# santi-pdp/segan_pytorch

Hardware: NVIDIA H100
Metric: 16384-sample windows/sec (G+D train step) (higher is better)
Workload: dtype f16 operands / f32 accumulate (f16 gradient tensors, loss scale 1024)

## Files before the change

include/segan_b200.h:

```cpp
#ifndef SEGAN_B200_H
#define SEGAN_B200_H

#include <stdint.h>

#ifdef __cplusplus
extern "C" {
#endif

#define SG_ABI_VERSION 3

#define SG_STAT_SLICES 8

#define SG_OK 0
#define SG_ERR_INVALID -1
#define SG_ERR_LAUNCH -2
#define SG_ERR_UNSUPPORTED -3

#define SG_F32 0
#define SG_F16 1
#define SG_BF16 2

#define SG_ACT_NONE 0
#define SG_ACT_PRELU 1
#define SG_ACT_TANH 2
// ... 33 lines not shown
  int32_t n_lo, n_hi;
  const float* bias;
  int32_t bias_mod;
  int32_t batch;
  int32_t ksplit;
  int32_t backend;
  int32_t tile_n;
  double* bn_stats;
  void* out2;
  int32_t out2_halo;
  const float* slope;
  int32_t slope_mod;
  void* sk_ws;
} sg_tapgemm_f;

int sg_tapgemm_f_run(const sg_tapgemm_f* p, void* stream);
int64_t sg_tapgemm_f_workspace_bytes(void);
int sg_debug_timeline(unsigned long long* host_out, int max_words);

typedef struct sg_tapgemm_w {
  const void* g;
  int32_t g_rows, g_dtype;
  const void* a0;
  const void* a1;
  int32_t a0_c, a1_c;
  int32_t a_rows, a_halo, a_dtype;
  int32_t kc, nc;
  int32_t d_lo, d_hi;
  int32_t tap_k_lo[9], tap_k_hi[9], tap_n_lo[9], tap_n_hi[9];
  float* dw;
// ... 134 lines not shown
```

segan_pytorch_b200/csrc/tapgemm_tc.cu:

```cuda
#include "common.cuh"
#include <cuda.h>
#include <stdlib.h>

namespace sg {

__device__ __forceinline__ uint32_t smem_u32(const void* p) {
  return static_cast<uint32_t>(__cvta_generic_to_shared(p));
}
__device__ __forceinline__ void mbar_init(uint64_t* bar, uint32_t count) {
  asm volatile("mbarrier.init.shared::cta.b64 [%0], %1;" ::"r"(smem_u32(bar)), "r"(count));
}
__device__ __forceinline__ void mbar_expect_tx(uint64_t* bar, uint32_t bytes) {
  asm volatile("mbarrier.arrive.expect_tx.shared::cta.b64 _, [%0], %1;" ::"r"(smem_u32(bar)), "r"(bytes)
               : "memory");
}
__device__ __forceinline__ void mbar_arrive(uint64_t* bar) {
  asm volatile("mbarrier.arrive.shared::cta.b64 _, [%0];" ::"r"(smem_u32(bar)) : "memory");
}
__device__ __forceinline__ uint32_t mbar_try(uint32_t addr, uint32_t parity) {
  uint32_t done;
  asm volatile(
      "{\n"
      ".reg .pred p;\n"
      "mbarrier.try_wait.parity.shared::cta.b64 p, [%1], %2;\n"
// ... 52 lines not shown
  asm volatile("ld.shared.v4.b32 {%0, %1, %2, %3}, [%4];" : "=r"(v.x), "=r"(v.y), "=r"(v.z), "=r"(v.w) : "r"(addr) : "memory");
  return v;
}
__device__ __forceinline__ void red_add_v2(float* addr, float a, float b) {
  asm volatile("red.global.add.v2.f32 [%0], {%1, %2};" ::"l"(addr), "f"(a), "f"(b) : "memory");
}
__device__ __forceinline__ void wgmma_fence() { asm volatile("wgmma.fence.sync.aligned;" ::: "memory"); }
__device__ __forceinline__ void wgmma_commit() { asm volatile("wgmma.commit_group.sync.aligned;" ::: "memory"); }
template <int N>
__device__ __forceinline__ void wgmma_wait() { asm volatile("wgmma.wait_group.sync.aligned %0;" ::"n"(N) : "memory"); }
template <int R>
__device__ __forceinline__ void setmaxnreg_inc() { asm volatile("setmaxnreg.inc.sync.aligned.u32 %0;" ::"n"(R)); }
template <int R>
__device__ __forceinline__ void setmaxnreg_dec() { asm volatile("setmaxnreg.dec.sync.aligned.u32 %0;" ::"n"(R)); }
__device__ __forceinline__ void consumer_bar_sync() { asm volatile("bar.sync 1, 256;" ::: "memory"); }

template <int TA, int TB>
__device__ __forceinline__ void wgmma_f16_n64(float (&d)[32], uint64_t da, uint64_t db, int scale_d) {
  asm volatile(
      "{\n.reg .pred p;\nsetp.ne.b32 p, %34, 0;\n"
      "wgmma.mma_async.sync.aligned.m64n64k16.f32.f16.f16 "
      "{%0, %1, %2, %3, %4, %5, %6, %7, %8, %9, %10, %11, %12, %13, %14, %15, %16, %17, %18, %19, %20, %21, %22, %23, %24, %25, %26, %27, %28, %29, %30, %31}, %32, %33, p, 1, 1, %35, %36;\n}\n"
      : "+f"(d[0]), "+f"(d[1]), "+f"(d[2]), "+f"(d[3]), "+f"(d[4]), "+f"(d[5]), "+f"(d[6]), "+f"(d[7]), "+f"(d[8]), "+f"(d[9]), "+f"(d[10]), "+f"(d[11]), "+f"(d[12]), "+f"(d[13]), "+f"(d[14]), "+f"(d[15]), "+f"(d[16]), "+f"(d[17]), "+f"(d[18]), "+f"(d[19]), "+f"(d[20]), "+f"(d[21]), "+f"(d[22]), "+f"(d[23]), "+f"(d[24]), "+f"(d[25]), "+f"(d[26]), "+f"(d[27]), "+f"(d[28]), "+f"(d[29]), "+f"(d[30]), "+f"(d[31])
      : "l"(da), "l"(db), "r"(scale_d), "n"(TA), "n"(TB));
}

template <int TA, int TB>
__device__ __forceinline__ void wgmma_bf16_n64(float (&d)[32], uint64_t da, uint64_t db, int scale_d) {
  asm volatile(
      "{\n.reg .pred p;\nsetp.ne.b32 p, %34, 0;\n"
// ... 65 lines not shown
  d |= (uint64_t)((sbo_bytes >> 4) & 0x3FFF) << 32;
  d |= (uint64_t)1 << 62;
  return d;
}

template <int N, int TA, int TB, bool BF16>
__device__ __forceinline__ void mma_k64(float (&acc)[N / 2], uint64_t da, uint64_t db, uint32_t a_step,
                                        uint32_t b_step, bool first) {
  wgmma_fence();
#pragma unroll
  for (int kk = 0; kk < 4; ++kk)
    wgmma_tile<N, TA, TB, BF16>(acc, da + kk * a_step, db + kk * b_step, (first && kk == 0) ? 0 : 1);
  wgmma_commit();
}

constexpr int STAGES = 4;
constexpr int A_STAGE_BYTES = 128 * 128;
constexpr int B_STAGE_BYTES = 256 * 128;
constexpr int STAGE_BYTES = A_STAGE_BYTES + B_STAGE_BYTES;
constexpr int SMEM_BYTES = STAGES * STAGE_BYTES + 1024  + 256  + 2048 ;
constexpr int OUT_CHUNK_BYTES = 128 * 128;
constexpr int OUT_STAGE_OFF = STAGES * STAGE_BYTES;
constexpr int F_CTL_OFF = OUT_STAGE_OFF + 2 * OUT_CHUNK_BYTES;
constexpr int F_SMEM_BYTES = F_CTL_OFF + 256  + 1024 ;
static_assert(F_SMEM_BYTES <= 232448, "form-F shared memory exceeds the sm_90 opt-in limit");
constexpr int NUM_THREADS = 384;
constexpr int PRODUCER_REGS = 40, CONSUMER_REGS = 232;

struct TapRangesTC {
  int k_lo[NTAP], k_hi[NTAP], n_lo[NTAP], n_hi[NTAP];
};

struct FTcParams {
  int a0_c, kc, nc, a_halo;
  int d_lo, d_hi;
  TapRangesTC tr;
  void* out; int out_dtype, out_rows, out_halo, out_ld, out_col0;
  int w_tap0;
  int m_lo, m_hi, n_lo;
  const float* bias; int bias_mod;
  int batch, ksplit;
  int TR, TB, TN;
  int m_tiles_per_b, b_tiles, n_tiles;
  int dbg;
  double* stats;
  int sk_dp_tiles;
  int sk_split;
  float* sk_ws;
  unsigned int* sk_cnt;
  void* out2;
  int out2_halo;
  const float* slope; int slope_mod;
  int bias_mask, slope_mask;
  int tma_out;
};

struct SharedCtl {
  uint64_t full[STAGES];
  uint64_t empty[STAGES];
};

__device__ __forceinline__ int f_num_steps(const FTcParams& p, int n0, int ks) {
  int total = 0;
  for (int d = p.d_lo; d <= p.d_hi; ++d) {
    const int ti = d + 4;
    if (n0 + p.TN <= p.tr.n_lo[ti] || n0 >= p.tr.n_hi[ti]) continue;
    total += (p.tr.k_hi[ti] - p.tr.k_lo[ti]) >> 6;
  }
  return p.ksplit == 1 ? total : (total - ks + p.ksplit - 1) / p.ksplit;
}

struct Piece {
  int tile;
  int mt, rest;
  int kb, ke;
  int total;
};

constexpr int TL_SLOTS = 32;
constexpr int TL_CTAS = 160;
__device__ unsigned long long g_tc_timeline[TL_CTAS * TL_SLOTS];
__device__ __forceinline__ unsigned long long gtime_ns() {
  unsigned long long t;
  asm volatile("mov.u64 %0, %globaltimer;" : "=l"(t));
  return t;
}

struct PieceIter {
  int m_tiles, nctas, dp_end, total_tiles, cta;
  int next_dp, cur_mt, cur_rest;
  int cache_rest, cache_steps;
  bool sk_done;

  __device__ __forceinline__ int steps_of_rest(const FTcParams& p, int rest) {
    if (rest != cache_rest) {
      cache_rest = rest;
// ... 132 lines not shown
        sx += __shfl_xor_sync(0xffffffffu, sx, o);
        sy += __shfl_xor_sync(0xffffffffu, sy, o);
        qx += __shfl_xor_sync(0xffffffffu, qx, o);
        qy += __shfl_xor_sync(0xffffffffu, qy, o);
      }
      if (lane < 4) {
        atomicAdd(colstat + c, sx);
        atomicAdd(colstat + c + 1, sy);
        atomicAdd(colstat + 256 + c, qx);
        atomicAdd(colstat + 256 + c + 1, qy);
      }
    }
  }
}

template <int TN>
__device__ __forceinline__ void f_epilogue_tma(const FTcParams& p, const float (&acc)[TN / 2], int mt, int n0,
                                               int ctid, uint32_t stg, const CUtensorMap* tmO,
                                               const CUtensorMap* tmO2) {
  const int lane = ctid & 31, cw = ctid >> 5;
  const int mtb = p.m_tiles_per_b == 1 ? mt : mt / p.m_tiles_per_b;
  const int b0 = mtb * p.TB;
  const int m0 = p.m_lo + (mt - mtb * p.m_tiles_per_b) * p.TR;
  const bool two = p.out2 != nullptr;
  const bool act_in_place = p.slope != nullptr && !two;
  const bool add_bias = p.bias != nullptr;
  const uint32_t row_off = (uint32_t)(cw * 16 + (lane >> 2)) * 128u + 4u * (lane & 3);
  const int sw = lane >> 2;
  const int halo2 = p.out2_halo;
  const bool mirror_tile = two && halo2 > 0 &&
                           ((m0 <= halo2 && m0 + p.TR > 1) || (m0 + p.TR > p.out_rows - 1 - halo2 && m0 <= p.out_rows - 2));
  constexpr int NQ = TN / 64;
#pragma unroll
  for (int q = 0; q < NQ; ++q) {
    const bool round_start = two || (q & 1) == 0;
    const bool round_end = two || (q & 1) == 1 || q == NQ - 1;
    const uint32_t slot = stg + (two ? 0u : (uint32_t)(q & 1) * OUT_CHUNK_BYTES);
    if (round_start) {
      if (ctid == 0) bulk_wait_read_all();
      consumer_bar_sync();
    }
#pragma unroll
    for (int jj = 0; jj < 8; ++jj) {
      const int j = 8 * q + jj;
      const int c = 8 * j + 2 * (lane & 3);
      float bx = 0.f, by = 0.f;
      if (add_bias) {
        const float* bp = p.bias + f_mod(n0 + c, p.bias_mod, p.bias_mask);
        bx = __ldg(bp); by = __ldg(bp + 1);
      }
      float s0 = 0.f, s1 = 0.f;
      if (p.slope != nullptr) {
        const float* sp = p.slope + f_mod(n0 + c, p.slope_mod, p.slope_mask);
        s0 = __ldg(sp); s1 = __ldg(sp + 1);
      }
      const uint32_t col_off = (uint32_t)((jj ^ sw) << 4);
#pragma unroll
      for (int h = 0; h < 2; ++h) {
        float x = acc[4 * j + 2 * h] + bx, y = acc[4 * j + 2 * h + 1] + by;
        if (act_in_place) {
          x = x > 0.f ? x : s0 * x;
          y = y > 0.f ? y : s1 * y;
        }
        const uint32_t off = row_off + (uint32_t)h * 1024u + col_off;
        st_shared_u32(slot + off, pack2(x, y, p.out_dtype));
        if (two) st_shared_u32(slot + OUT_CHUNK_BYTES + off, pack2(x > 0.f ? x : s0 * x, y > 0.f ? y : s1 * y, p.out_dtype));
      }
    }
    if (!round_end) continue;
    fence_proxy_async_smem();
    consumer_bar_sync();
    if (ctid == 0) {
      const int c_rel = n0 - p.n_lo + 64 * q, m_rel = m0 - p.m_lo;
      if (two) {
        tma_store_3d(tmO, slot, c_rel, m_rel, b0);
        tma_store_3d(tmO2, slot + OUT_CHUNK_BYTES, c_rel, m_rel, b0);
      } else if (q & 1) {
        tma_store_3d(tmO, stg, c_rel - 64, m_rel, b0);
        tma_store_3d(tmO, stg + OUT_CHUNK_BYTES, c_rel, m_rel, b0);
      } else {
        tma_store_3d(tmO, stg, c_rel, m_rel, b0);
      }
      bulk_commit();
    }
    if (mirror_tile) {
      const int rows = p.TR * p.TB;
      const int out2_buf_rows = p.out_rows + 2 * halo2;
      for (int idx = ctid; idx < rows * 8; idx += 256) {
        const int r = idx >> 3, k = idx & 7;
        const int tb = r / p.TR, tr = r - tb * p.TR;
        const int b = b0 + tb, m = m0 + tr;
        if (b >= p.batch || m >= p.m_hi) continue;
        int mm;
        if (m >= 1 && m <= halo2) mm = -m;
        else if (m >= p.out_rows - 1 - halo2 && m <= p.out_rows - 2) mm = 2 * (p.out_rows - 1) - m;
        else continue;
        const uint4 v = ld_shared_v4(slot + OUT_CHUNK_BYTES + (uint32_t)r * 128u + (uint32_t)((k ^ (r & 7)) << 4));
        const int64_t o = ((int64_t)b * out2_buf_rows + halo2 + mm) * p.out_ld + p.out_col0 + (n0 - p.n_lo) + 64 * q + 8 * k;
        *reinterpret_cast<uint4*>(reinterpret_cast<uint16_t*>(p.out2) + o) = v;
      }
    }
  }
}

template <int TN, bool BF16>
__global__ void __launch_bounds__(NUM_THREADS, 1)
tapgemm_f_tc(const __grid_constant__ CUtensorMap tmA0, const __grid_constant__ CUtensorMap tmA1,
             const __grid_constant__ CUtensorMap tmW, const __grid_constant__ CUtensorMap tmO,
             const __grid_constant__ CUtensorMap tmO2, const FTcParams p) {
  extern __shared__ uint8_t smem_raw[];
  uint8_t* smem = reinterpret_cast<uint8_t*>((reinterpret_cast<uintptr_t>(smem_raw) + 1023) & ~uintptr_t(1023));
  SharedCtl* ctl = reinterpret_cast<SharedCtl*>(smem + F_CTL_OFF);
  float* colstat = reinterpret_cast<float*>(smem + OUT_STAGE_OFF);
  const int wg = threadIdx.x >> 7;

  if (threadIdx.x == 0) {
    prefetch_tmap(&tmA0); prefetch_tmap(&tmA1); prefetch_tmap(&tmW);
    if (p.tma_out) {
      prefetch_tmap(&tmO);
      if (p.out2 != nullptr) prefetch_tmap(&tmO2);
    }
    for (int s = 0; s < STAGES; ++s) { mbar_init(&ctl->full[s], 1); mbar_init(&ctl->empty[s], 2); }
    fence_barrier_init();
  }
  if (p.stats != nullptr)
    for (int c = threadIdx.x; c < 512; c += NUM_THREADS) colstat[c] = 0.f;
  __syncthreads();

  const int m_tiles = p.m_tiles_per_b * p.b_tiles;
  const int total_tiles = m_tiles * p.n_tiles * p.ksplit;
  const uint32_t a_bytes = (uint32_t)p.TR * p.TB * 128u;
  const uint32_t b_bytes = (uint32_t)TN * 128u;
  PieceIter it;
  it.init(p, m_tiles, total_tiles, blockIdx.x, gridDim.x);
  Piece pc;

  if (wg == 0) {
// ... 2 lines not shown
      int stage = 0; uint32_t phase = 0;
      while (it.next(p, pc)) {
        const int ks = p.ksplit == 1 ? 0 : pc.rest % p.ksplit;
        const int nt = p.ksplit == 1 ? pc.rest : pc.rest / p.ksplit;
        const int mtb = p.m_tiles_per_b == 1 ? pc.mt : pc.mt / p.m_tiles_per_b;
        const int b0 = mtb * p.TB;
        const int m0 = p.m_lo + (pc.mt - mtb * p.m_tiles_per_b) * p.TR;
        const int n0 = p.n_lo + nt * p.TN;
        const bool interleaved = p.ksplit > 1;
        int step = 0, sel = 0;
        int skip = interleaved ? 0 : pc.kb;
        int next_sel = ks;
        const int kstride = interleaved ? 64 * p.ksplit : 64;
        for (int d = p.d_lo; d <= p.d_hi; ++d) {
          const int ti = d + 4;
          if (n0 + p.TN <= p.tr.n_lo[ti] || n0 >= p.tr.n_hi[ti]) continue;
          const int klo = p.tr.k_lo[ti], khi = p.tr.k_hi[ti];
          const int nk = (khi - klo) >> 6;
          int k0 = klo;
          if (!interleaved) {
            if (skip >= nk) { skip -= nk; sel += nk; continue; }
            k0 += skip << 6; sel += skip; skip = 0;
            if (sel >= pc.ke) break;
          } else {
            if (next_sel >= step + nk) { step += nk; continue; }
            k0 += (next_sel - step) << 6;
          }
          for (; k0 < khi; k0 += kstride) {
            if (!interleaved) {
              if (sel++ >= pc.ke) break;
            } else {
              next_sel += p.ksplit;
            }
            mbar_wait(&ctl->empty[stage], phase ^ 1);
            uint8_t* sa = smem + stage * STAGE_BYTES;
            mbar_expect_tx(&ctl->full[stage], a_bytes + b_bytes);
            if (k0 < p.a0_c) tma_load_3d(sa, &tmA0, &ctl->full[stage], k0, m0 + d + p.a_halo, b0);
            else tma_load_3d(sa, &tmA1, &ctl->full[stage], k0 - p.a0_c, m0 + d + p.a_halo, b0);
            tma_load_2d(sa + A_STAGE_BYTES, &tmW, &ctl->full[stage], k0, (ti - p.w_tap0) * p.nc + n0);
            if (++stage == STAGES) { stage = 0; phase ^= 1; }
          }
          step += nk;
        }
      }
    }
    return;
  }

  setmaxnreg_inc<CONSUMER_REGS>();
  const int ctid = threadIdx.x - 128;
  const int cwg = wg - 1;
  const bool wg_leader = (threadIdx.x & 127) == 0;
  const uint32_t smem0 = smem_u32(smem);
  int stage = 0; uint32_t phase = 0;
  int stat_nt = -1;
  auto flush_stats = [&](int nt_done) {
    consumer_bar_sync();
    const int n0s = p.n_lo + nt_done * p.TN;
    double* o = p.stats + (int64_t)(blockIdx.x % SG_STAT_SLICES) * 2 * p.nc;
    for (int c = ctid; c < p.TN; c += 256) {
      atomicAdd(o + n0s + c, (double)colstat[c]);
      atomicAdd(o + p.nc + n0s + c, (double)colstat[256 + c]);
      colstat[c] = 0.f;
      colstat[256 + c] = 0.f;
    }
    consumer_bar_sync();
  };
  const bool tl_on = (p.dbg & (1 << 20)) && ctid == 0 && blockIdx.x < TL_CTAS;
  int tl_i = 0;
  unsigned long long* tl = g_tc_timeline + (blockIdx.x < TL_CTAS ? blockIdx.x : 0) * TL_SLOTS;
  if (tl_on) { for (int i = 0; i < TL_SLOTS; ++i) tl[i] = 0; tl[tl_i++] = gtime_ns(); }

  float acc[TN / 2];
  while (it.next(p, pc)) {
    const int ks = p.ksplit == 1 ? 0 : pc.rest % p.ksplit;
    const int nt = p.ksplit == 1 ? pc.rest : pc.rest / p.ksplit;
    const int n0 = p.n_lo + nt * p.TN;
    const bool partial = pc.tile >= it.dp_end;
    if (p.stats != nullptr && nt != stat_nt) {
      if (stat_nt >= 0) flush_stats(stat_nt);
      stat_nt = nt;
    }
    const int nsteps = pc.ke - pc.kb;
    if (nsteps == 0) {
#pragma unroll
      for (int j = 0; j < TN / 2; ++j) acc[j] = 0.f;
    }
    int prev = 0;
    for (int i = 0; i < nsteps; ++i) {
      mbar_wait(&ctl->full[stage], phase);
      const uint32_t sa = smem0 + (uint32_t)stage * STAGE_BYTES;
      mma_k64<TN, 0, 0, BF16>(acc, make_smem_desc(sa + (uint32_t)cwg * 8192u, 16, 1024),
                        make_smem_desc(sa + A_STAGE_BYTES, 16, 1024), 2, 2, i == 0);
      wgmma_wait<1>();
      if (i > 0 && wg_leader) mbar_arrive(&ctl->empty[prev]);
      prev = stage;
      if (++stage == STAGES) { stage = 0; phase ^= 1; }
    }
    wgmma_wait<0>();
    if (nsteps > 0 && wg_leader) mbar_arrive(&ctl->empty[prev]);
    if (tl_on && tl_i < TL_SLOTS - 1) tl[tl_i++] = gtime_ns();

    if (!partial) {
      if (p.tma_out) f_epilogue_tma<TN>(p, acc, pc.mt, n0, ctid, smem0 + OUT_STAGE_OFF, &tmO, &tmO2);
      else f_epilogue<TN>(p, acc, pc.mt, n0, ks, ctid, colstat);
      if (tl_on && tl_i < TL_SLOTS - 1) tl[tl_i++] = gtime_ns();
      continue;
    }
    constexpr int64_t SLOT_F2 = 128 * 256 / 2;
    float2* myslot = reinterpret_cast<float2*>(p.sk_ws) + (int64_t)blockIdx.x * SLOT_F2 + ctid;
#pragma unroll
    for (int j = 0; j < TN / 4; ++j) __stcg(myslot + j * 256, make_float2(acc[2 * j], acc[2 * j + 1]));
    if (tl_on && tl_i < TL_SLOTS - 1) tl[tl_i++] = gtime_ns();
    const int slot = pc.tile - it.dp_end;
    unsigned int* cnt = p.sk_cnt + slot * 8 + (ctid >> 5);
    __threadfence();
    __syncwarp();
    unsigned int old = 0;
    if ((ctid & 31) == 0) old = atomicAdd(cnt, 1u);
    old = __shfl_sync(0xffffffffu, old, 0);
    if (old + 1u == (unsigned int)p.sk_split) {
      __threadfence();
#pragma unroll
      for (int j = 0; j < TN / 2; ++j) acc[j] = 0.f;
      const float2* base0 = reinterpret_cast<const float2*>(p.sk_ws) + (int64_t)slot * p.sk_split * SLOT_F2 + ctid;
      for (int sp = 0; sp < p.sk_split; ++sp) {
#pragma unroll
        for (int j = 0; j < TN / 4; ++j) {
          const float2 t = __ldcg(base0 + sp * SLOT_F2 + j * 256);
          acc[2 * j] += t.x; acc[2 * j + 1] += t.y;
        }
      }
      f_epilogue<TN>(p, acc, pc.mt, n0, 0, ctid, colstat);
      __syncwarp();
      if ((ctid & 31) == 0) *cnt = 0u;
      if (tl_on && tl_i < TL_SLOTS - 1) tl[tl_i++] = gtime_ns() | (1ull << 63);
    }
  }
  if (tl_on && tl_i < TL_SLOTS) tl[tl_i++] = gtime_ns();
  if (p.stats != nullptr && stat_nt >= 0) flush_stats(stat_nt);
  if (p.tma_out && ctid == 0) bulk_wait_read_all();
}

struct WTcParams {
  int a0_c, kc, nc, a_halo;
  int d_lo, d_hi;
  TapRangesTC tr;
  float* dw; int dw_tap0;
// ... 179 lines not shown
                   strides, box, es, CU_TENSOR_MAP_INTERLEAVE_NONE, CU_TENSOR_MAP_SWIZZLE_128B,
                   CU_TENSOR_MAP_L2_PROMOTION_NONE, CU_TENSOR_MAP_FLOAT_OOB_FILL_NONE);
  if (r != CUDA_SUCCESS) {
    set_error("cuTensorMapEncodeTiled(store C=%d rows=%d B=%d ld=%d box=%d,%d) failed: %d", C, rows, B, ld, box_rows,
              box_b, (int)r);
    return SG_ERR_LAUNCH;
  }
  return SG_OK;
}

constexpr int SK_MAX_CTAS = 160;
constexpr int64_t SK_CNT_BYTES = 8192;
constexpr int64_t SK_WS_BYTES = SK_CNT_BYTES + (int64_t)SK_MAX_CTAS * 128 * 256 * 4;
int64_t tapgemm_f_workspace_bytes() { return SK_WS_BYTES; }
int tapgemm_f_debug_timeline(unsigned long long* host_out, int max_words) {
  const int n = max_words < TL_CTAS * TL_SLOTS ? max_words : TL_CTAS * TL_SLOTS;
  if (cudaMemcpyFromSymbol(host_out, g_tc_timeline, (size_t)n * sizeof(unsigned long long)) != cudaSuccess) return -1;
  return n;
}
int g_stream_k = [] { const char* e = getenv("SEGAN_B200_STREAMK"); return e ? atoi(e) : 16; }();
double g_sk_atomic_steps = [] { const char* e = getenv("SEGAN_B200_SK_ATOMIC"); return e ? atof(e) : 4.5; }();
double g_sk_fixed_steps = [] { const char* e = getenv("SEGAN_B200_SK_FIXED"); return e ? atof(e) : 60.0; }();

int g_cta_pair = 1;

static int num_sms() {
  static int n = 0;
  if (n == 0) {
    int dev = 0;
    cudaGetDevice(&dev);
    cudaDeviceGetAttribute(&n, cudaDevAttrMultiProcessorCount, dev);
// ... 15 lines not shown
    p.tr.n_lo[i] = q->tap_n_lo[i]; p.tr.n_hi[i] = q->tap_n_hi[i];
  }
  p.out = q->out; p.out_dtype = q->out_dtype; p.out_rows = q->out_rows; p.out_halo = q->out_halo;
  p.out_ld = q->out_ld > 0 ? q->out_ld : q->nc;
  p.out_col0 = q->out_ld > 0 ? q->out_col0 : q->n_lo;
  p.w_tap0 = q->w_tap0;
  p.m_lo = q->m_lo; p.m_hi = q->m_hi; p.n_lo = q->n_lo;
  p.bias = q->bias; p.bias_mod = q->bias_mod > 0 ? q->bias_mod : q->nc;
  p.batch = q->batch; p.ksplit = q->ksplit < 1 ? 1 : q->ksplit;
  const int rows_m = q->m_hi - q->m_lo;
  const int ncols = q->n_hi - q->n_lo;
  if (rows_m >= 128) { p.TR = 128; p.TB = 1; }
  else { p.TR = rows_m; p.TB = 128 / rows_m; if (p.TB > q->batch) p.TB = q->batch; }
  p.m_tiles_per_b = (rows_m + p.TR - 1) / p.TR;
  p.b_tiles = (q->batch + p.TB - 1) / p.TB;
  p.TN = (ncols % 256 == 0) ? 256 : (ncols % 128 == 0 ? 128 : 64);
  if ((q->tile_n == 64 || q->tile_n == 128 || q->tile_n == 256) && ncols % q->tile_n == 0 && q->tile_n < p.TN)
    p.TN = q->tile_n;
  p.n_tiles = ncols / p.TN;
  {
    static const int dbg_env = [] { const char* e = getenv("SEGAN_B200_DEBUG"); return e ? atoi(e) : 0; }();
    p.dbg = dbg_env;
  }
  p.stats = q->bn_stats;
  p.sk_dp_tiles = 0x7fffffff; p.sk_split = 1; p.sk_ws = nullptr; p.sk_cnt = nullptr;
  p.out2 = q->out2; p.out2_halo = q->out2_halo; p.slope = q->slope; p.slope_mod = q->slope_mod;
  p.bias_mask = (p.bias_mod & (p.bias_mod - 1)) == 0 ? p.bias_mod - 1 : -1;
  p.slope_mask = (p.slope_mod > 0 && (p.slope_mod & (p.slope_mod - 1)) == 0) ? p.slope_mod - 1 : -1;
  if (q->bn_stats != nullptr) SG_CHECK_ARG(p.ksplit == 1 && q->out_dtype != SG_F32 && q->n_lo == 0 && q->n_hi == q->nc);
  CUtensorMap tmA0, tmA1, tmW;
  const int a_buf_rows = q->a_rows + 2 * q->a_halo;
  int rc = make_map3(&tmA0, q->a0, q->a_dtype, q->a0_c, a_buf_rows, q->batch, p.TR, p.TB);
  if (rc) return rc;
  if (q->a1) rc = make_map3(&tmA1, q->a1, q->a_dtype, q->a1_c, a_buf_rows, q->batch, p.TR, p.TB);
  else tmA1 = tmA0;
  if (rc) return rc;
  rc = make_map2(&tmW, q->w, q->w_dtype, q->kc, (int64_t)(q->d_hi + 4 - q->w_tap0 + 1) * q->nc, p.TN);
  if (rc) return rc;
  const int tiles = p.m_tiles_per_b * p.b_tiles * p.n_tiles * p.ksplit;
  int nctas = num_sms();
  if (tiles < nctas) nctas = tiles;
  if (q->sk_ws != nullptr && g_stream_k > 1 && p.ksplit == 1 && q->bn_stats == nullptr && nctas <= SK_MAX_CTAS &&
      tiles > nctas && tiles % nctas != 0) {
    const int r = tiles % nctas;
    int steps = 0;
    for (int d = q->d_lo; d <= q->d_hi; ++d) steps += (q->tap_k_hi[d + 4] - q->tap_k_lo[d + 4]) / 64;
    int best_s = 1;
    double best = (double)steps;
    int s_max = nctas / r < g_stream_k ? nctas / r : g_stream_k;
    if (s_max > steps / 2) s_max = steps / 2;
    const double per_partial = g_sk_atomic_steps * 256.0 / p.TN;
    for (int S = 2; S <= s_max; ++S) {
      const double c = (double)steps / S + per_partial * S + g_sk_fixed_steps;
      if (c < best) { best = c; best_s = S; }
    }
    const bool split = best_s > 1 && best < 0.92 * steps && steps >= 2 * best_s;
    static const bool verbose = getenv("SEGAN_B200_SK_VERBOSE") != nullptr;
    if (verbose)
      fprintf(stderr, "tapgemm_f split-K: %d tiles on %d CTAs, %d left over, %d k-steps, TN %d -> split %d\n",
              tiles, nctas, r, steps, p.TN, split ? best_s : 1);
    if (split) {
      p.sk_dp_tiles = (tiles / nctas) * nctas;
      p.sk_split = best_s;
      p.sk_cnt = reinterpret_cast<unsigned int*>(q->sk_ws);
      p.sk_ws = reinterpret_cast<float*>(reinterpret_cast<uint8_t*>(q->sk_ws) + SK_CNT_BYTES);
    }
  }
  p.tma_out = q->out_dtype != SG_F32 && q->bn_stats == nullptr;
  CUtensorMap tmO = tmA0, tmO2 = tmA0;
  if (p.tma_out) {
    rc = make_store_map3(&tmO, q->out, q->out_dtype, ncols, rows_m, q->batch, p.out_ld, q->out_rows + 2 * q->out_halo,
                         q->out_halo + q->m_lo, p.out_col0, p.TR, p.TB);
    if (rc) return rc;
    if (q->out2 != nullptr) {
      rc = make_store_map3(&tmO2, q->out2, q->out_dtype, ncols, rows_m, q->batch, p.out_ld,
                           q->out_rows + 2 * q->out2_halo, q->out2_halo + q->m_lo, p.out_col0, p.TR, p.TB);
      if (rc) return rc;
    }
  }
  const bool bf = q->a_dtype == SG_BF16;
  void (*kern)(CUtensorMap, CUtensorMap, CUtensorMap, CUtensorMap, CUtensorMap, FTcParams);
  if (p.TN == 256) kern = bf ? tapgemm_f_tc<256, true> : tapgemm_f_tc<256, false>;
  else if (p.TN == 128) kern = bf ? tapgemm_f_tc<128, true> : tapgemm_f_tc<128, false>;
  else kern = bf ? tapgemm_f_tc<64, true> : tapgemm_f_tc<64, false>;
  SG_CHECK_CUDA(cudaFuncSetAttribute(kern, cudaFuncAttributeMaxDynamicSharedMemorySize, F_SMEM_BYTES));
  void* args[] = {&tmA0, &tmA1, &tmW, &tmO, &tmO2, &p};
  SG_CHECK_CUDA(cudaLaunchKernel(reinterpret_cast<const void*>(kern), dim3(nctas), dim3(NUM_THREADS), args,
                                 (size_t)F_SMEM_BYTES, st));
  return SG_OK;
}

template <typename K>
static int launch_persistent(K kern, int grid, const CUtensorMap& t0, const CUtensorMap& t1, const CUtensorMap& t2,
                             const void* params, cudaStream_t st) {
  SG_CHECK_CUDA(cudaFuncSetAttribute(kern, cudaFuncAttributeMaxDynamicSharedMemorySize, SMEM_BYTES));
  void* args[] = {const_cast<CUtensorMap*>(&t0), const_cast<CUtensorMap*>(&t1), const_cast<CUtensorMap*>(&t2),
                  const_cast<void*>(params)};
  SG_CHECK_CUDA(cudaLaunchKernel(reinterpret_cast<const void*>(kern), dim3(grid), dim3(NUM_THREADS), args,
                                 (size_t)SMEM_BYTES, st));
  return SG_OK;
}

int tapgemm_w_tc_launch(const sg_tapgemm_w* q, cudaStream_t st) {
// ... 38 lines not shown
```

segan_pytorch_b200/engine.py:

```python
import ctypes as C
import math
import os

import torch

from . import _lib
from ._lib import (ACT_NONE, ACT_PRELU, BACKEND_FFMA, BACKEND_TCGEN05, SG_BF16, SG_DHEAD_CONV, SG_DHEAD_GAVG,
                   SG_DHEAD_GMAX, SG_DHEAD_MLP, SG_F16, SG_F32, TapGemmF, TapGemmW)

KW = 31
DHEAD_KINDS = {"conv": SG_DHEAD_CONV, "gmax": SG_DHEAD_GMAX, "gavg": SG_DHEAD_GAVG, "mlp": SG_DHEAD_MLP}


def wave_on_tensor_cores():
    return os.environ.get("SEGAN_B200_WAVE", "tc").lower() not in ("cuda", "ffma", "0")


def wave_col_weights(w, dev):
    wc = torch.zeros(w.shape[0], 2, 32, dtype=torch.float32, device=dev)
    wc[:, :w.shape[1], :KW] = w
    return wc.view(w.shape[0], 64)


_DEC_LAST_KIDX = None
# ... 178 lines not shown
    waves = -(-tiles // pairs_hw)
    rem = tiles % pairs_hw
    if tiles <= pairs_hw or rem == 0 or waves > 10:
        return batch, 0
    per_gran = _f_tiling(rows_m, gran, ncols)[3]
    full_tiles = (tiles // pairs_hw) * pairs_hw
    b1 = min(batch, (full_tiles // per_gran) * gran)
    if b1 <= 0 or b1 >= batch:
        return batch, 0
    tail_tiles = _f_tiling(rows_m, batch - b1, ncols)[3]
    s = min(pairs_hw // max(1, tail_tiles), ksteps // 4, 32)
    if s < 2:
        return batch, 0
    return b1, s


_SK_WS = {}
STREAM_K = os.environ.get("SEGAN_B200_STREAMK", "1").lower() not in ("0", "off", "no", "false")


def sk_workspace(dev):
    if not STREAM_K:
        return None
    idx = torch.device(dev).index
    key = (torch.cuda.current_device() if idx is None else idx, torch.cuda.current_stream().cuda_stream)
    ws = _SK_WS.get(key)
    if ws is None:
        ws = _SK_WS[key] = torch.zeros(int(_lib.load().sg_tapgemm_f_workspace_bytes()), dtype=torch.uint8, device=dev)
    return ws

# ... 34 lines not shown
        q.a0_c, q.a1_c = a0_c, a1_c
        q.a_rows, q.a_halo, q.a_dtype = a_rows, a_halo, a_dtype
        q.w, q.w_dtype, q.w_tap0 = _p(w), w_dtype, w_tap0
        q.kc, q.nc, q.d_lo, q.d_hi = kc, nc, d_lo, d_hi
        for i in range(9):
            q.tap_k_lo[i], q.tap_k_hi[i], q.tap_n_lo[i], q.tap_n_hi[i] = taps[0][i], taps[1][i], taps[2][i], taps[3][i]
        if tail:
            q.out = _p(ws)
        else:
            q.out = _p(out) if b_off == 0 else C.c_void_p(out.data_ptr() + b_off * out_brows * old * esz)
        q.out_ld, q.out_col0 = out_ld, out_col0
        q.out_dtype, q.out_rows, q.out_halo = (SG_F32 if tail else out_dtype), out_rows, out_halo
        q.m_lo, q.m_hi, q.n_lo, q.n_hi = m_lo, m_hi, n_lo, n_hi
        q.bias, q.bias_mod = _p(bias), bias_mod
        q.batch, q.ksplit = nb, (tail_ks if tail else ksplit)
        q.backend, q.tile_n = backend, tn
        q.bn_stats = _p(stats)
        assert (out2 is None and slope is None) or b1 == batch, "fused activation outputs are not split"
        q.out2, q.out2_halo, q.slope, q.slope_mod = _p(out2), out2_halo, _p(slope), slope_mod
        q.sk_ws = _p(sk_workspace(out.device)) if backend == BACKEND_TCGEN05 else None
        with _Prof("tapgemm_f", _tap_flops(taps, d_lo, d_hi, q.n_lo, q.n_hi, (m_hi - m_lo) * nb)):
            _lib.call("sg_tapgemm_f_run", C.byref(q), _stream())
        if tail:
            col_lo = out_col0 if out_ld > 0 else n_lo
            _lib.call("sg_convert_f32_rows", _p(ws), C.c_void_p(out.data_ptr() + b_off * out_brows * old * esz),
                      out_dtype, nb * out_brows, old, col_lo, n_hi - n_lo, _stream())


def run_w(g, g_rows, g_dtype, a0, a1, a_rows, a_halo, a_dtype, kc, nc, taps, dw, batch, d_lo=-4, d_hi=4,
          dw_tap0=0, ksplit=1, backend=None, a0_c=None, a1_c=0, out_scale=None):
    q = TapGemmW()
# ... 1575 lines not shown
```

Before: 9982.

## Add ping-pong warpgroup schedule to forward tap-GEMM with TN=128 auto-selection

Adds a ping-pong variant of the forward tap-GEMM kernel. The two consumer warpgroups alternate whole output tiles, each computing a full 128-row tile with two m64 wgmma accumulators, and ordered named barriers let one warpgroup's epilogue overlap the other's mainloop. The variant uses 5 smaller pipeline stages and per-warpgroup output staging. The host now auto-drops TN from 256 to 128 when wave fill is poor or K is short, and selects ping-pong by default when TN<=128, TMA output is on and no split-K is planned. The cost is doubled accumulator registers per warpgroup and more tiles at TN=128, which reloads A more often.

```diff
diff --git a/include/segan_b200.h b/include/segan_b200.h
--- a/include/segan_b200.h
+++ b/include/segan_b200.h
@@ -71,6 +71,8 @@
   void* sk_ws;
 } sg_tapgemm_f;
 
+#define SG_TILE_COOPERATIVE 0x10000
+#define SG_TILE_PINGPONG 0x20000
 int sg_tapgemm_f_run(const sg_tapgemm_f* p, void* stream);
 int64_t sg_tapgemm_f_workspace_bytes(void);
 int sg_debug_timeline(unsigned long long* host_out, int max_words);
diff --git a/segan_pytorch_b200/csrc/tapgemm_tc.cu b/segan_pytorch_b200/csrc/tapgemm_tc.cu
--- a/segan_pytorch_b200/csrc/tapgemm_tc.cu
+++ b/segan_pytorch_b200/csrc/tapgemm_tc.cu
@@ -90,6 +90,12 @@
 template <int R>
 __device__ __forceinline__ void setmaxnreg_dec() { asm volatile("setmaxnreg.dec.sync.aligned.u32 %0;" ::"n"(R)); }
 __device__ __forceinline__ void consumer_bar_sync() { asm volatile("bar.sync 1, 256;" ::: "memory"); }
+__device__ __forceinline__ void named_bar_sync(int id, int n) {
+  asm volatile("bar.sync %0, %1;" ::"r"(id), "r"(n) : "memory");
+}
+__device__ __forceinline__ void named_bar_arrive(int id, int n) {
+  asm volatile("bar.arrive %0, %1;" ::"r"(id), "r"(n) : "memory");
+}
 
 template <int TA, int TB>
 __device__ __forceinline__ void wgmma_f16_n64(float (&d)[32], uint64_t da, uint64_t db, int scale_d) {
@@ -185,6 +191,17 @@
   wgmma_commit();
 }
 
+template <int N, bool BF16>
+__device__ __forceinline__ void mma_k64_m128(float (&acc)[2][N / 2], uint64_t da, uint64_t db, bool first) {
+  wgmma_fence();
+#pragma unroll
+  for (int kk = 0; kk < 4; ++kk)
+#pragma unroll
+    for (int hm = 0; hm < 2; ++hm)
+      wgmma_tile<N, 0, 0, BF16>(acc[hm], da + hm * 512 + kk * 2, db + kk * 2, (first && kk == 0) ? 0 : 1);
+  wgmma_commit();
+}
+
 constexpr int STAGES = 4;
 constexpr int A_STAGE_BYTES = 128 * 128;
 constexpr int B_STAGE_BYTES = 256 * 128;
@@ -195,6 +212,14 @@
 constexpr int F_CTL_OFF = OUT_STAGE_OFF + 2 * OUT_CHUNK_BYTES;
 constexpr int F_SMEM_BYTES = F_CTL_OFF + 256  + 1024 ;
 static_assert(F_SMEM_BYTES <= 232448, "form-F shared memory exceeds the sm_90 opt-in limit");
+constexpr int PP_STAGES = 5;
+constexpr int PP_STAGE_BYTES = A_STAGE_BYTES + 128 * 128;
+constexpr int PP_OUT_STAGE_OFF = PP_STAGES * PP_STAGE_BYTES;
+constexpr int PP_CTL_OFF = PP_OUT_STAGE_OFF + 2 * 2 * OUT_CHUNK_BYTES;
+constexpr int PP_SMEM_BYTES = PP_CTL_OFF + 256  + 1024 ;
+static_assert(PP_SMEM_BYTES <= 232448, "form-F ping-pong shared memory exceeds the sm_90 opt-in limit");
+static_assert(PP_STAGES >= STAGES, "SharedCtl holds PP_STAGES barrier pairs");
+constexpr int PP_ORDER_BAR = 2, PP_EPI_BAR = 4;
 constexpr int NUM_THREADS = 384;
 constexpr int PRODUCER_REGS = 40, CONSUMER_REGS = 232;
 
@@ -224,18 +249,24 @@
   const float* slope; int slope_mod;
   int bias_mask, slope_mask;
   int tma_out;
+  int skip_n;
 };
 
 struct SharedCtl {
-  uint64_t full[STAGES];
-  uint64_t empty[STAGES];
+  uint64_t full[PP_STAGES];
+  uint64_t empty[PP_STAGES];
 };
+
+__device__ __forceinline__ bool f_tap_misses(const FTcParams& p, int n0, int ti) {
+  const int s0 = n0 - (n0 - p.n_lo) % p.skip_n;
+  return s0 + p.skip_n <= p.tr.n_lo[ti] || s0 >= p.tr.n_hi[ti];
+}
 
 __device__ __forceinline__ int f_num_steps(const FTcParams& p, int n0, int ks) {
   int total = 0;
   for (int d = p.d_lo; d <= p.d_hi; ++d) {
     const int ti = d + 4;
-    if (n0 + p.TN <= p.tr.n_lo[ti] || n0 >= p.tr.n_hi[ti]) continue;
+    if (f_tap_misses(p, n0, ti)) continue;
     total += (p.tr.k_hi[ti] - p.tr.k_lo[ti]) >> 6;
   }
   return p.ksplit == 1 ? total : (total - ks + p.ksplit - 1) / p.ksplit;
@@ -250,7 +281,8 @@
 
 constexpr int TL_SLOTS = 32;
 constexpr int TL_CTAS = 160;
-__device__ unsigned long long g_tc_timeline[TL_CTAS * TL_SLOTS];
+constexpr unsigned long long TL_MAINLOOP = 1ull << 62;
+__device__ unsigned long long g_tc_timeline[2 * TL_CTAS * TL_SLOTS];
 __device__ __forceinline__ unsigned long long gtime_ns() {
   unsigned long long t;
   asm volatile("mov.u64 %0, %globaltimer;" : "=l"(t));
@@ -413,11 +445,12 @@
   }
 }
 
-template <int TN>
-__device__ __forceinline__ void f_epilogue_tma(const FTcParams& p, const float (&acc)[TN / 2], int mt, int n0,
-                                               int ctid, uint32_t stg, const CUtensorMap* tmO,
-                                               const CUtensorMap* tmO2) {
-  const int lane = ctid & 31, cw = ctid >> 5;
+template <int TN, int MH>
+__device__ __forceinline__ void f_epilogue_tma(const FTcParams& p, const float (&acc)[MH][TN / 2], int mt, int n0,
+                                               int et, uint32_t stg, const CUtensorMap* tmO,
+                                               const CUtensorMap* tmO2, int bar_id) {
+  constexpr int NT = 256 / MH;
+  const int lane = et & 31, cw = et >> 5;
   const int mtb = p.m_tiles_per_b == 1 ? mt : mt / p.m_tiles_per_b;
   const int b0 = mtb * p.TB;
   const int m0 = p.m_lo + (mt - mtb * p.m_tiles_per_b) * p.TR;
@@ -436,8 +469,8 @@
     const bool round_end = two || (q & 1) == 1 || q == NQ - 1;
     const uint32_t slot = stg + (two ? 0u : (uint32_t)(q & 1) * OUT_CHUNK_BYTES);
     if (round_start) {
-      if (ctid == 0) bulk_wait_read_all();
-      consumer_bar_sync();
+      if (et == 0) bulk_wait_read_all();
+      named_bar_sync(bar_id, NT);
     }
 #pragma unroll
     for (int jj = 0; jj < 8; ++jj) {
@@ -455,21 +488,23 @@
       }
       const uint32_t col_off = (uint32_t)((jj ^ sw) << 4);
 #pragma unroll
+      for (int hm = 0; hm < MH; ++hm)
+#pragma unroll
       for (int h = 0; h < 2; ++h) {
-        float x = acc[4 * j + 2 * h] + bx, y = acc[4 * j + 2 * h + 1] + by;
+        float x = acc[hm][4 * j + 2 * h] + bx, y = acc[hm][4 * j + 2 * h + 1] + by;
         if (act_in_place) {
           x = x > 0.f ? x : s0 * x;
           y = y > 0.f ? y : s1 * y;
         }
-        const uint32_t off = row_off + (uint32_t)h * 1024u + col_off;
+        const uint32_t off = row_off + (uint32_t)hm * 8192u + (uint32_t)h * 1024u + col_off;
         st_shared_u32(slot + off, pack2(x, y, p.out_dtype));
         if (two) st_shared_u32(slot + OUT_CHUNK_BYTES + off, pack2(x > 0.f ? x : s0 * x, y > 0.f ? y : s1 * y, p.out_dtype));
       }
     }
     if (!round_end) continue;
     fence_proxy_async_smem();
-    consumer_bar_sync();
-    if (ctid == 0) {
+    named_bar_sync(bar_id, NT);
+    if (et == 0) {
       const int c_rel = n0 - p.n_lo + 64 * q, m_rel = m0 - p.m_lo;
       if (two) {
         tma_store_3d(tmO, slot, c_rel, m_rel, b0);
@@ -485,7 +520,7 @@
     if (mirror_tile) {
       const int rows = p.TR * p.TB;
       const int out2_buf_rows = p.out_rows + 2 * halo2;
-      for (int idx = ctid; idx < rows * 8; idx += 256) {
+      for (int idx = et; idx < rows * 8; idx += NT) {
         const int r = idx >> 3, k = idx & 7;
         const int tb = r / p.TR, tr = r - tb * p.TR;
         const int b = b0 + tb, m = m0 + tr;
@@ -502,14 +537,17 @@
   }
 }
 
-template <int TN, bool BF16>
+template <int TN, bool BF16, bool PP>
 __global__ void __launch_bounds__(NUM_THREADS, 1)
 tapgemm_f_tc(const __grid_constant__ CUtensorMap tmA0, const __grid_constant__ CUtensorMap tmA1,
              const __grid_constant__ CUtensorMap tmW, const __grid_constant__ CUtensorMap tmO,
              const __grid_constant__ CUtensorMap tmO2, const FTcParams p) {
+  static_assert(!PP || TN <= 128, "ping-pong accumulators: TN <= 128");
+  constexpr int NST = PP ? PP_STAGES : STAGES;
+  constexpr int SB = PP ? PP_STAGE_BYTES : STAGE_BYTES;
   extern __shared__ uint8_t smem_raw[];
   uint8_t* smem = reinterpret_cast<uint8_t*>((reinterpret_cast<uintptr_t>(smem_raw) + 1023) & ~uintptr_t(1023));
-  SharedCtl* ctl = reinterpret_cast<SharedCtl*>(smem + F_CTL_OFF);
+  SharedCtl* ctl = reinterpret_cast<SharedCtl*>(smem + (PP ? PP_CTL_OFF : F_CTL_OFF));
   float* colstat = reinterpret_cast<float*>(smem + OUT_STAGE_OFF);
   const int wg = threadIdx.x >> 7;
 
@@ -519,7 +557,7 @@
       prefetch_tmap(&tmO);
       if (p.out2 != nullptr) prefetch_tmap(&tmO2);
     }
-    for (int s = 0; s < STAGES; ++s) { mbar_init(&ctl->full[s], 1); mbar_init(&ctl->empty[s], 2); }
+    for (int s = 0; s < NST; ++s) { mbar_init(&ctl->full[s], 1); mbar_init(&ctl->empty[s], PP ? 1 : 2); }
     fence_barrier_init();
   }
   if (p.stats != nullptr)
@@ -552,7 +590,7 @@
         const int kstride = interleaved ? 64 * p.ksplit : 64;
         for (int d = p.d_lo; d <= p.d_hi; ++d) {
           const int ti = d + 4;
-          if (n0 + p.TN <= p.tr.n_lo[ti] || n0 >= p.tr.n_hi[ti]) continue;
+          if (f_tap_misses(p, n0, ti)) continue;
           const int klo = p.tr.k_lo[ti], khi = p.tr.k_hi[ti];
           const int nk = (khi - klo) >> 6;
           int k0 = klo;
@@ -571,12 +609,12 @@
               next_sel += p.ksplit;
             }
             mbar_wait(&ctl->empty[stage], phase ^ 1);
-            uint8_t* sa = smem + stage * STAGE_BYTES;
+            uint8_t* sa = smem + stage * SB;
             mbar_expect_tx(&ctl->full[stage], a_bytes + b_bytes);
             if (k0 < p.a0_c) tma_load_3d(sa, &tmA0, &ctl->full[stage], k0, m0 + d + p.a_halo, b0);
             else tma_load_3d(sa, &tmA1, &ctl->full[stage], k0 - p.a0_c, m0 + d + p.a_halo, b0);
             tma_load_2d(sa + A_STAGE_BYTES, &tmW, &ctl->full[stage], k0, (ti - p.w_tap0) * p.nc + n0);
-            if (++stage == STAGES) { stage = 0; phase ^= 1; }
+            if (++stage == NST) { stage = 0; phase ^= 1; }
           }
           step += nk;
         }
@@ -591,6 +629,56 @@
   const bool wg_leader = (threadIdx.x & 127) == 0;
   const uint32_t smem0 = smem_u32(smem);
   int stage = 0; uint32_t phase = 0;
+
+  if constexpr (PP) {
+    const int et = threadIdx.x & 127;
+    const uint32_t stg = smem0 + PP_OUT_STAGE_OFF + (uint32_t)cwg * 2u * OUT_CHUNK_BYTES;
+    const bool tl_on = (p.dbg & (1 << 20)) && et == 0 && blockIdx.x < TL_CTAS;
+    int tl_i = 0;
+    unsigned long long* tl = g_tc_timeline + ((size_t)cwg * TL_CTAS + (blockIdx.x < TL_CTAS ? blockIdx.x : 0)) * TL_SLOTS;
+    if (tl_on) { for (int i = 0; i < TL_SLOTS; ++i) tl[i] = 0; tl[tl_i++] = gtime_ns(); }
+    float acc[2][TN / 2];
+    int idx = 0;
+    bool more = it.next(p, pc);
+    while (more) {
+      const int mt = pc.mt, n0 = p.n_lo + pc.rest * p.TN, nsteps = pc.ke - pc.kb;
+      more = it.next(p, pc);
+      if ((idx++ & 1) != cwg) {
+        const int s = stage + nsteps;
+        phase ^= (uint32_t)((s / NST) & 1);
+        stage = s % NST;
+        continue;
+      }
+      if (idx > 1) named_bar_sync(PP_ORDER_BAR + cwg, 256);
+      if (tl_on && tl_i < TL_SLOTS - 1) tl[tl_i++] = gtime_ns() | TL_MAINLOOP;
+      if (nsteps == 0) {
+#pragma unroll
+        for (int hm = 0; hm < 2; ++hm)
+#pragma unroll
+          for (int j = 0; j < TN / 2; ++j) acc[hm][j] = 0.f;
+      }
+      int prev = 0;
+      for (int i = 0; i < nsteps; ++i) {
+        mbar_wait(&ctl->full[stage], phase);
+        const uint32_t sa = smem0 + (uint32_t)stage * SB;
+        mma_k64_m128<TN, BF16>(acc, make_smem_desc(sa, 16, 1024), make_smem_desc(sa + A_STAGE_BYTES, 16, 1024), i == 0);
+        wgmma_wait<1>();
+        if (i > 0 && wg_leader) mbar_arrive(&ctl->empty[prev]);
+        prev = stage;
+        if (++stage == NST) { stage = 0; phase ^= 1; }
+      }
+      if (more) named_bar_arrive(PP_ORDER_BAR + (cwg ^ 1), 256);
+      wgmma_wait<0>();
+      if (nsteps > 0 && wg_leader) mbar_arrive(&ctl->empty[prev]);
+      if (tl_on && tl_i < TL_SLOTS - 1) tl[tl_i++] = gtime_ns();
+      f_epilogue_tma<TN, 2>(p, acc, mt, n0, et, stg, &tmO, &tmO2, PP_EPI_BAR + cwg);
+      if (tl_on && tl_i < TL_SLOTS - 1) tl[tl_i++] = gtime_ns();
+    }
+    if (tl_on && tl_i < TL_SLOTS) tl[tl_i++] = gtime_ns();
+    if (et == 0) bulk_wait_read_all();
+    return;
+  }
+
   int stat_nt = -1;
   auto flush_stats = [&](int nt_done) {
     consumer_bar_sync();
@@ -607,9 +695,12 @@
   const bool tl_on = (p.dbg & (1 << 20)) && ctid == 0 && blockIdx.x < TL_CTAS;
   int tl_i = 0;
   unsigned long long* tl = g_tc_timeline + (blockIdx.x < TL_CTAS ? blockIdx.x : 0) * TL_SLOTS;
-  if (tl_on) { for (int i = 0; i < TL_SLOTS; ++i) tl[i] = 0; tl[tl_i++] = gtime_ns(); }
-
-  float acc[TN / 2];
+  if (tl_on) {
+    for (int i = 0; i < TL_SLOTS; ++i) tl[i] = tl[TL_CTAS * TL_SLOTS + i] = 0;
+    tl[tl_i++] = gtime_ns();
+  }
+
+  float acc[1][TN / 2];
   while (it.next(p, pc)) {
     const int ks = p.ksplit == 1 ? 0 : pc.rest % p.ksplit;
     const int nt = p.ksplit == 1 ? pc.rest : pc.rest / p.ksplit;
@@ -622,13 +713,13 @@
     const int nsteps = pc.ke - pc.kb;
     if (nsteps == 0) {
 #pragma unroll
-      for (int j = 0; j < TN / 2; ++j) acc[j] = 0.f;
+      for (int j = 0; j < TN / 2; ++j) acc[0][j] = 0.f;
     }
     int prev = 0;
     for (int i = 0; i < nsteps; ++i) {
       mbar_wait(&ctl->full[stage], phase);
       const uint32_t sa = smem0 + (uint32_t)stage * STAGE_BYTES;
-      mma_k64<TN, 0, 0, BF16>(acc, make_smem_desc(sa + (uint32_t)cwg * 8192u, 16, 1024),
+      mma_k64<TN, 0, 0, BF16>(acc[0], make_smem_desc(sa + (uint32_t)cwg * 8192u, 16, 1024),
                         make_smem_desc(sa + A_STAGE_BYTES, 16, 1024), 2, 2, i == 0);
       wgmma_wait<1>();
       if (i > 0 && wg_leader) mbar_arrive(&ctl->empty[prev]);
@@ -640,15 +731,15 @@
     if (tl_on && tl_i < TL_SLOTS - 1) tl[tl_i++] = gtime_ns();
 
     if (!partial) {
-      if (p.tma_out) f_epilogue_tma<TN>(p, acc, pc.mt, n0, ctid, smem0 + OUT_STAGE_OFF, &tmO, &tmO2);
-      else f_epilogue<TN>(p, acc, pc.mt, n0, ks, ctid, colstat);
+      if (p.tma_out) f_epilogue_tma<TN, 1>(p, acc, pc.mt, n0, ctid, smem0 + OUT_STAGE_OFF, &tmO, &tmO2, 1);
+      else f_epilogue<TN>(p, acc[0], pc.mt, n0, ks, ctid, colstat);
       if (tl_on && tl_i < TL_SLOTS - 1) tl[tl_i++] = gtime_ns();
       continue;
     }
     constexpr int64_t SLOT_F2 = 128 * 256 / 2;
     float2* myslot = reinterpret_cast<float2*>(p.sk_ws) + (int64_t)blockIdx.x * SLOT_F2 + ctid;
 #pragma unroll
-    for (int j = 0; j < TN / 4; ++j) __stcg(myslot + j * 256, make_float2(acc[2 * j], acc[2 * j + 1]));
+    for (int j = 0; j < TN / 4; ++j) __stcg(myslot + j * 256, make_float2(acc[0][2 * j], acc[0][2 * j + 1]));
     if (tl_on && tl_i < TL_SLOTS - 1) tl[tl_i++] = gtime_ns();
     const int slot = pc.tile - it.dp_end;
     unsigned int* cnt = p.sk_cnt + slot * 8 + (ctid >> 5);
@@ -660,16 +751,16 @@
     if (old + 1u == (unsigned int)p.sk_split) {
       __threadfence();
 #pragma unroll
-      for (int j = 0; j < TN / 2; ++j) acc[j] = 0.f;
+      for (int j = 0; j < TN / 2; ++j) acc[0][j] = 0.f;
       const float2* base0 = reinterpret_cast<const float2*>(p.sk_ws) + (int64_t)slot * p.sk_split * SLOT_F2 + ctid;
       for (int sp = 0; sp < p.sk_split; ++sp) {
 #pragma unroll
         for (int j = 0; j < TN / 4; ++j) {
           const float2 t = __ldcg(base0 + sp * SLOT_F2 + j * 256);
-          acc[2 * j] += t.x; acc[2 * j + 1] += t.y;
+          acc[0][2 * j] += t.x; acc[0][2 * j + 1] += t.y;
         }
       }
-      f_epilogue<TN>(p, acc, pc.mt, n0, 0, ctid, colstat);
+      f_epilogue<TN>(p, acc[0], pc.mt, n0, 0, ctid, colstat);
       __syncwarp();
       if ((ctid & 31) == 0) *cnt = 0u;
       if (tl_on && tl_i < TL_SLOTS - 1) tl[tl_i++] = gtime_ns() | (1ull << 63);
@@ -879,7 +970,7 @@
 constexpr int64_t SK_WS_BYTES = SK_CNT_BYTES + (int64_t)SK_MAX_CTAS * 128 * 256 * 4;
 int64_t tapgemm_f_workspace_bytes() { return SK_WS_BYTES; }
 int tapgemm_f_debug_timeline(unsigned long long* host_out, int max_words) {
-  const int n = max_words < TL_CTAS * TL_SLOTS ? max_words : TL_CTAS * TL_SLOTS;
+  const int n = max_words < 2 * TL_CTAS * TL_SLOTS ? max_words : 2 * TL_CTAS * TL_SLOTS;
   if (cudaMemcpyFromSymbol(host_out, g_tc_timeline, (size_t)n * sizeof(unsigned long long)) != cudaSuccess) return -1;
   return n;
 }
@@ -925,10 +1016,12 @@
   else { p.TR = rows_m; p.TB = 128 / rows_m; if (p.TB > q->batch) p.TB = q->batch; }
   p.m_tiles_per_b = (rows_m + p.TR - 1) / p.TR;
   p.b_tiles = (q->batch + p.TB - 1) / p.TB;
+  const int sched = q->tile_n & (SG_TILE_COOPERATIVE | SG_TILE_PINGPONG);
+  const int tile_n = q->tile_n & ~(SG_TILE_COOPERATIVE | SG_TILE_PINGPONG);
+  SG_CHECK_ARG(sched != (SG_TILE_COOPERATIVE | SG_TILE_PINGPONG));
   p.TN = (ncols % 256 == 0) ? 256 : (ncols % 128 == 0 ? 128 : 64);
-  if ((q->tile_n == 64 || q->tile_n == 128 || q->tile_n == 256) && ncols % q->tile_n == 0 && q->tile_n < p.TN)
-    p.TN = q->tile_n;
-  p.n_tiles = ncols / p.TN;
+  if ((tile_n == 64 || tile_n == 128 || tile_n == 256) && ncols % tile_n == 0 && tile_n < p.TN)
+    p.TN = tile_n;
   {
     static const int dbg_env = [] { const char* e = getenv("SEGAN_B200_DEBUG"); return e ? atoi(e) : 0; }();
     p.dbg = dbg_env;
@@ -939,6 +1032,39 @@
   p.bias_mask = (p.bias_mod & (p.bias_mod - 1)) == 0 ? p.bias_mod - 1 : -1;
   p.slope_mask = (p.slope_mod > 0 && (p.slope_mod & (p.slope_mod - 1)) == 0) ? p.slope_mod - 1 : -1;
   if (q->bn_stats != nullptr) SG_CHECK_ARG(p.ksplit == 1 && q->out_dtype != SG_F32 && q->n_lo == 0 && q->n_hi == q->nc);
+  p.tma_out = q->out_dtype != SG_F32 && q->bn_stats == nullptr;
+
+  int steps = 0;
+  for (int d = q->d_lo; d <= q->d_hi; ++d) steps += (q->tap_k_hi[d + 4] - q->tap_k_lo[d + 4]) / 64;
+  auto tiles_of = [&](int tn) { return p.m_tiles_per_b * p.b_tiles * (ncols / tn) * p.ksplit; };
+  auto ctas_of = [&](int tn) { return tiles_of(tn) < num_sms() ? tiles_of(tn) : num_sms(); };
+  auto split_of = [&](int tn) {
+    const int tiles = tiles_of(tn), nctas = ctas_of(tn);
+    if (q->sk_ws == nullptr || g_stream_k <= 1 || p.ksplit != 1 || q->bn_stats != nullptr || nctas > SK_MAX_CTAS ||
+        tiles <= nctas || tiles % nctas == 0)
+      return 1;
+    const int r = tiles % nctas;
+    int best_s = 1;
+    double best = (double)steps;
+    int s_max = nctas / r < g_stream_k ? nctas / r : g_stream_k;
+    if (s_max > steps / 2) s_max = steps / 2;
+    const double per_partial = g_sk_atomic_steps * 256.0 / tn;
+    for (int S = 2; S <= s_max; ++S) {
+      const double c = (double)steps / S + per_partial * S + g_sk_fixed_steps;
+      if (c < best) { best = c; best_s = S; }
+    }
+    return best_s > 1 && best < 0.92 * steps && steps >= 2 * best_s ? best_s : 1;
+  };
+  p.skip_n = p.TN;
+  if (sched == 0 && tile_n == 0 && p.TN == 256 && p.tma_out && p.ksplit == 1 && split_of(256) == 1 &&
+      split_of(128) == 1) {
+    auto fill = [&](int tn) {
+      const int t = tiles_of(tn), c = ctas_of(tn);
+      return (double)t / ((double)((t + c - 1) / c) * c);
+    };
+    if (steps <= 24 || (fill(256) < 0.85 && fill(128) >= fill(256) + 0.1)) p.TN = 128;
+  }
+  p.n_tiles = ncols / p.TN;
   CUtensorMap tmA0, tmA1, tmW;
   const int a_buf_rows = q->a_rows + 2 * q->a_halo;
   int rc = make_map3(&tmA0, q->a0, q->a_dtype, q->a0_c, a_buf_rows, q->batch, p.TR, p.TB);
@@ -948,36 +1074,19 @@
   if (rc) return rc;
   rc = make_map2(&tmW, q->w, q->w_dtype, q->kc, (int64_t)(q->d_hi + 4 - q->w_tap0 + 1) * q->nc, p.TN);
   if (rc) return rc;
-  const int tiles = p.m_tiles_per_b * p.b_tiles * p.n_tiles * p.ksplit;
-  int nctas = num_sms();
-  if (tiles < nctas) nctas = tiles;
-  if (q->sk_ws != nullptr && g_stream_k > 1 && p.ksplit == 1 && q->bn_stats == nullptr && nctas <= SK_MAX_CTAS &&
-      tiles > nctas && tiles % nctas != 0) {
-    const int r = tiles % nctas;
-    int steps = 0;
-    for (int d = q->d_lo; d <= q->d_hi; ++d) steps += (q->tap_k_hi[d + 4] - q->tap_k_lo[d + 4]) / 64;
-    int best_s = 1;
-    double best = (double)steps;
-    int s_max = nctas / r < g_stream_k ? nctas / r : g_stream_k;
-    if (s_max > steps / 2) s_max = steps / 2;
-    const double per_partial = g_sk_atomic_steps * 256.0 / p.TN;
-    for (int S = 2; S <= s_max; ++S) {
-      const double c = (double)steps / S + per_partial * S + g_sk_fixed_steps;
-      if (c < best) { best = c; best_s = S; }
-    }
-    const bool split = best_s > 1 && best < 0.92 * steps && steps >= 2 * best_s;
-    static const bool verbose = getenv("SEGAN_B200_SK_VERBOSE") != nullptr;
-    if (verbose)
-      fprintf(stderr, "tapgemm_f split-K: %d tiles on %d CTAs, %d left over, %d k-steps, TN %d -> split %d\n",
-              tiles, nctas, r, steps, p.TN, split ? best_s : 1);
-    if (split) {
-      p.sk_dp_tiles = (tiles / nctas) * nctas;
-      p.sk_split = best_s;
-      p.sk_cnt = reinterpret_cast<unsigned int*>(q->sk_ws);
-      p.sk_ws = reinterpret_cast<float*>(reinterpret_cast<uint8_t*>(q->sk_ws) + SK_CNT_BYTES);
-    }
-  }
-  p.tma_out = q->out_dtype != SG_F32 && q->bn_stats == nullptr;
+  const int tiles = tiles_of(p.TN);
+  const int nctas = ctas_of(p.TN);
+  const int best_s = split_of(p.TN);
+  static const bool verbose = getenv("SEGAN_B200_SK_VERBOSE") != nullptr;
+  if (verbose && tiles > nctas && tiles % nctas != 0)
+    fprintf(stderr, "tapgemm_f split-K: %d tiles on %d CTAs, %d left over, %d k-steps, TN %d -> split %d\n", tiles,
+            nctas, tiles % nctas, steps, p.TN, best_s);
+  if (best_s > 1) {
+    p.sk_dp_tiles = (tiles / nctas) * nctas;
+    p.sk_split = best_s;
+    p.sk_cnt = reinterpret_cast<unsigned int*>(q->sk_ws);
+    p.sk_ws = reinterpret_cast<float*>(reinterpret_cast<uint8_t*>(q->sk_ws) + SK_CNT_BYTES);
+  }
   CUtensorMap tmO = tmA0, tmO2 = tmA0;
   if (p.tma_out) {
     rc = make_store_map3(&tmO, q->out, q->out_dtype, ncols, rows_m, q->batch, p.out_ld, q->out_rows + 2 * q->out_halo,
@@ -989,15 +1098,27 @@
       if (rc) return rc;
     }
   }
+  const bool pp_ok = p.TN <= 128 && p.tma_out && p.ksplit == 1;
+  const bool split_planned = p.sk_dp_tiles < tiles;
+  if (sched == SG_TILE_PINGPONG) SG_CHECK_ARG(pp_ok && !split_planned);
+  const bool pp = sched == SG_TILE_PINGPONG || (sched == 0 && pp_ok && !split_planned);
   const bool bf = q->a_dtype == SG_BF16;
   void (*kern)(CUtensorMap, CUtensorMap, CUtensorMap, CUtensorMap, CUtensorMap, FTcParams);
-  if (p.TN == 256) kern = bf ? tapgemm_f_tc<256, true> : tapgemm_f_tc<256, false>;
-  else if (p.TN == 128) kern = bf ? tapgemm_f_tc<128, true> : tapgemm_f_tc<128, false>;
-  else kern = bf ? tapgemm_f_tc<64, true> : tapgemm_f_tc<64, false>;
-  SG_CHECK_CUDA(cudaFuncSetAttribute(kern, cudaFuncAttributeMaxDynamicSharedMemorySize, F_SMEM_BYTES));
+  if (pp) {
+    if (p.TN == 128) kern = bf ? tapgemm_f_tc<128, true, true> : tapgemm_f_tc<128, false, true>;
+    else kern = bf ? tapgemm_f_tc<64, true, true> : tapgemm_f_tc<64, false, true>;
+  } else if (p.TN == 256) {
+    kern = bf ? tapgemm_f_tc<256, true, false> : tapgemm_f_tc<256, false, false>;
+  } else if (p.TN == 128) {
+    kern = bf ? tapgemm_f_tc<128, true, false> : tapgemm_f_tc<128, false, false>;
+  } else {
+    kern = bf ? tapgemm_f_tc<64, true, false> : tapgemm_f_tc<64, false, false>;
+  }
+  const int smem_bytes = pp ? PP_SMEM_BYTES : F_SMEM_BYTES;
+  SG_CHECK_CUDA(cudaFuncSetAttribute(kern, cudaFuncAttributeMaxDynamicSharedMemorySize, smem_bytes));
   void* args[] = {&tmA0, &tmA1, &tmW, &tmO, &tmO2, &p};
   SG_CHECK_CUDA(cudaLaunchKernel(reinterpret_cast<const void*>(kern), dim3(nctas), dim3(NUM_THREADS), args,
-                                 (size_t)F_SMEM_BYTES, st));
+                                 (size_t)smem_bytes, st));
   return SG_OK;
 }
 
diff --git a/segan_pytorch_b200/engine.py b/segan_pytorch_b200/engine.py
--- a/segan_pytorch_b200/engine.py
+++ b/segan_pytorch_b200/engine.py
@@ -216,6 +216,8 @@
         return batch, 0
     return b1, s
 
+
+F_SCHEDULE = 0
 
 _SK_WS = {}
 STREAM_K = os.environ.get("SEGAN_B200_STREAMK", "1").lower() not in ("0", "off", "no", "false")
@@ -280,7 +282,7 @@
         q.m_lo, q.m_hi, q.n_lo, q.n_hi = m_lo, m_hi, n_lo, n_hi
         q.bias, q.bias_mod = _p(bias), bias_mod
         q.batch, q.ksplit = nb, (tail_ks if tail else ksplit)
-        q.backend, q.tile_n = backend, tn
+        q.backend, q.tile_n = backend, tn | F_SCHEDULE
         q.bn_stats = _p(stats)
         assert (out2 is None and slope is None) or b1 == batch, "fused activation outputs are not split"
         q.out2, q.out2_halo, q.slope, q.slope_mod = _p(out2), out2_halo, _p(slope), slope_mod
```

After: 10220, median of 6. 1.02x the previous value.
